# aproposorg/sydr

Measured on AMD Instinct MI355X. Metric: IQ Msamples/s through 32-ch E/P/L correlators @25 MHz fs, higher is better.
Workload: dtype f64

## Files before the change

sydr_amd/csrc/correlator_chip.h:

```cpp
#pragma once

#include "correlator.h"

#pragma clang fp contract(off)

namespace sdr {

constexpr int kChipMax = 26;
constexpr double kChipMinCodeStep = 1.0 / 25.9;
constexpr double kChipMaxCodeStep = 1.0 / 15.5;
constexpr int kChipRawDwords = 13;
constexpr int kChipRotSlots = 2 * kChipMax + 2;
template <int NT>
constexpr int chip_strip_slots() { return 2 * NT + 1; }

__host__ __device__ __forceinline__ int chip_first_above(double thr, double shift, double inv_step, bool& near) {
    const double u = (thr - shift) * inv_step;
    const double fl = floor(u);
    const double fr = u - fl;
    near = near || fr < kNearInteger || fr > 1.0 - kNearInteger;
    return (int)fl + 1;
}
__host__ __device__ __forceinline__ int chip_first_above_exact(int c, double thr, double step, double shift) {
    auto above = [&](int i) {
        double y = (double)i * step;
        y = y + shift;
        return y > thr;
    };
    if (c >= 1 && above(c - 1)) return (c >= 2 && above(c - 2)) ? c - 2 : c - 1;
    if (c < 0) c = 0;
    if (above(c)) return c;
    return above(c + 1) ? c + 1 : c + 2;
}

template <int B, int E, class F>
__device__ __forceinline__ void static_for(F&& f) {
    if constexpr (B < E) {
        f(std::integral_constant<int, B>{});
        static_for<B + 1, E>(f);
    }
}

__device__ __forceinline__ int wave_min_i32(int x) {
#pragma unroll
    for (int off = 1; off < 64; off <<= 1) {
        const int o = __shfl_xor(x, off, 64);
        x = o < x ? o : x;
    }
    return __builtin_amdgcn_readfirstlane(x);
}

#ifndef SDR_BIASED_CVT
#define SDR_BIASED_CVT 1
#endif
constexpr double kCvtBias = 4224.0;
#ifndef SDR_ALT_PAIRS
#define SDR_ALT_PAIRS 1
#endif
typedef uint32_t sdr_u32x2 __attribute__((ext_vector_type(2)));
__device__ __forceinline__ double biased_sample(sdr_u32x2& pair, uint32_t w_flipped, uint32_t selector, uint32_t hi_const) {
    pair.y = __builtin_amdgcn_perm(w_flipped, hi_const, selector);
    return __builtin_bit_cast(double, pair);
}
constexpr uint32_t cvt_selector(int byte) { return 0x03020000u | ((uint32_t)(4 + byte) << 8) | 0x0Cu; }

template <int NT>
struct ChipGeom {
    int64_t Tfx, Ufx;
    uint64_t delta[NT];
    int q0, F;
    int head_end, tail_start;
    int m[NT], J[NT];
    int bad;
};

template <int NT, int KM, int KS, int KI>
__host__ __device__ __forceinline__ void chip_geometry(int n, const double* shift, const double* step, const double* inv_step,
                                                       ChipGeom<NT>& g) {
    constexpr int A = NT / 2;
    const double two32 = 4294967296.0;
    g.q0 = (int)ceil(shift[A]);
    double y_last = (double)(n - 1) * step[A];
    y_last = y_last + shift[A];
    const int q_last = (int)ceil(y_last);
    g.F = q_last - g.q0 - 1;
    g.head_end = n, g.tail_start = n;
    if (g.F > 0) {
        bool nr = false;
        g.head_end = chip_first_above_exact(chip_first_above((double)g.q0, shift[A], inv_step[A], nr), (double)g.q0, step[A], shift[A]);
        g.tail_start = chip_first_above_exact(chip_first_above((double)(q_last - 1), shift[A], inv_step[A], nr),
                                              (double)(q_last - 1), step[A], shift[A]);
    }
    g.Tfx = (int64_t)rint(inv_step[A] * two32);
    g.Ufx = (int64_t)floor(-shift[A] * inv_step[A] * two32);
    const int M = (int)(g.Tfx >> 32);
    bool bad = M < 1 || M + 1 > kChipMax || g.F > 16384 || (KM != 0 && M != KM);
#pragma unroll
    for (int t = 0; t < NT; ++t) {
        g.m[t] = M, g.J[t] = 0, g.delta[t] = 0;
        if (t == A) continue;
        const int64_t Ut = (int64_t)floor(-shift[t] * inv_step[t] * two32);
        int j = (int)ceil(shift[t] - shift[A]) - 1;
        int64_t d = (Ut - g.Ufx) + (int64_t)(1 + j) * g.Tfx;
        if (d < 0) {
            d += g.Tfx;
            ++j;
        } else if (d >= g.Tfx) {
            d -= g.Tfx;
            --j;
        }
        bad = bad || d < 0 || d >= g.Tfx;
        g.J[t] = j;
        g.delta[t] = (uint64_t)d;
        g.m[t] = (int)(d >> 32);
        bad = bad || (KS != 0 && (g.m[t] != KS || j != (t < A ? -1 : 0)));
        bad = bad || (KI != 0 && !((j == (t - A) * KI - 1 && g.m[t] == 0) || (j == (t - A) * KI && g.m[t] >= M)));
    }
    g.bad = bad ? 1 : 0;
}

constexpr int kStaticHalf = 13;
constexpr int chip_half(int KM, int KS, int KI) { return KI != 0 ? (KM + 2) / 2 : KS + 1; }
struct ChipRot {
    double urc[kStaticHalf + 1], urs[kStaticHalf + 1];
    double rd0c, rd0s, rd1c, rd1s;
    double biasc[3], biass[3];
};
__host__ __device__ inline void chip_rotations(double dphi, int Dmin, ChipRot& r, int half = kStaticHalf, int cmin = kStaticHalf - 2) {
    double cs[16], sn[16];
    for (int k = 0; k < 16; ++k) sincos_reduced(-(double)k * dphi, &sn[k], &cs[k]);
    for (int k = 1; k <= half; ++k) r.urc[k] = cs[k], r.urs[k] = sn[k];
    r.urc[0] = 1.0, r.urs[0] = 0.0;
    sincos_reduced(-(double)Dmin * dphi, &r.rd0s, &r.rd0c);
    sincos_reduced(-(double)(Dmin + 1) * dphi, &r.rd1s, &r.rd1c);
    for (int st = 1; st < 16; st <<= 1)
        for (int l = 15; l >= st; --l) cs[l] += cs[l - st], sn[l] += sn[l - st];
    for (int i = 0; i < 3; ++i) {
        const int l = cmin + i - 1;
        const double re = cs[l] - sn[l], im = cs[l] + sn[l];
        r.biasc[i] = re * 4224.0, r.biass[i] = im * 4224.0;
    }
}

template <int NT>
struct ChipSetup {
    double dphi;
    double shift[NT], step[NT], inv_step[NT];
    int64_t base;
    ChipGeom<NT> g;
    ChipRot r;
};

template <int NT, int KM, int KS, int KI>
__host__ __device__ inline void chip_setup(int n, int64_t start_sample, int64_t capacity, double carrier_hz, double rem_code,
                                           double code_step, const double* spacing, double fs, int stride, ChipSetup<NT>& S) {
    S = ChipSetup<NT>{};
    S.dphi = carrier_step(carrier_hz, fs);
    const double nd = (double)n;
    for (int t = 0; t < NT; ++t) {
        const double shift = rem_code + spacing[t];
        double stop = code_step * nd;
        stop = stop + shift;
        const double delta = stop - shift;
        S.shift[t] = shift;
        S.step[t] = delta / nd;
        S.inv_step[t] = 1.0 / S.step[t];
    }
    const int64_t base = start_sample % capacity;
    const bool applies = code_step >= kChipMinCodeStep && code_step <= kChipMaxCodeStep && base + n + 32 <= capacity;
    S.base = applies ? base : -1;
    if (applies) {
        chip_geometry<NT, KM, KS, KI>(n, S.shift, S.step, S.inv_step, S.g);
        chip_rotations(S.dphi, (int)(((int64_t)stride * S.g.Tfx) >> 32), S.r, chip_half(KM, KS, KI), KM - chip_half(KM, KS, KI));
    }
}

struct ChipWalk {
    int S;
    uint32_t f;
};
__host__ __device__ __forceinline__ ChipWalk chip_walk_at(uint64_t u) { return ChipWalk{(int)(u >> 32), (uint32_t)u}; }
__host__ __device__ __forceinline__ bool chip_carry(uint32_t a, uint32_t b, uint32_t& sum) { return __builtin_add_overflow(a, b, &sum); }
__host__ __device__ __forceinline__ bool chip_near_sample(uint32_t fr) { return fr + 0x10000u < 0x20000u; }
__host__ __device__ __forceinline__ bool chip_walk_step(ChipWalk& w, uint32_t stride_lo, int Dmin) {
    const bool dd = chip_carry(w.f, stride_lo, w.f);
    w.S = w.S + Dmin + (dd ? 1 : 0);
    return dd;
}
__host__ __device__ __forceinline__ ChipWalk chip_walk_clamp(const ChipWalk& w, bool inside, const ChipWalk& w_last) {
    return ChipWalk{inside ? w.S : w_last.S, inside ? w.f : w_last.f};
}
template <int NT, int KI>
__host__ __device__ __forceinline__ void chip_walk_flags(uint32_t f, uint32_t T_lo, const uint32_t* delta_lo, bool& dn, bool* ds, bool& near) {
    uint32_t fE;
    dn = chip_carry(f, T_lo, fE);
    near = chip_near_sample(f) || chip_near_sample(fE);
#pragma unroll
    for (int t = 0; t < NT; ++t) {
        ds[t] = false;
        if (t == NT / 2 || KI != 0) continue;
        uint32_t fT;
        ds[t] = chip_carry(f, delta_lo[t], fT);
        near = near || chip_near_sample(fT);
    }
}

template <int NT>
struct ChipBlock {
    uint32_t raw[kChipRawDwords];
    int S;
    int dn;
    int ds[NT];
    uint32_t f;
    int slow;
    int adj;
};

template <int NT, bool SINGLE_WAVE, int KM = 0, int KS = 0, int KI = 0>
__device__ __forceinline__ bool correlate_epoch_chip(const void* __restrict__ ring, const void* __restrict__ ring_flipped, int64_t capacity,
                                                     const EpochParams& ep, double dphi, const EpochConsts<NT>& K,
                                                     const ChipGeom<NT>& G, int64_t base, const ChipRot* R,
                                                     const uint32_t* lut, double2* strip_lds, double2* rot, int tid,
                                                     int lane, int stride, int edge_lane, double* accr, double* acci) {
    constexpr int A = NT / 2;
    constexpr int kSlots = chip_strip_slots<NT>();
    const int n = ep.n;
    const double* shift = K.shift;
    const double* step = K.step;
    double2* strip = strip_lds + tid * kSlots;
    const int wlane = threadIdx.x & 63;
#pragma unroll
    for (int t = 0; t < NT; ++t) accr[t] = acci[t] = 0.0;

    const double dphi_u = uniform(dphi), rem_carrier_u = uniform(ep.rem_carrier);
    const int q0 = __builtin_amdgcn_readfirstlane(G.q0);
    const int F = __builtin_amdgcn_readfirstlane(G.F);
    const int head_end = __builtin_amdgcn_readfirstlane(G.head_end);
    const int tail_start = __builtin_amdgcn_readfirstlane(G.tail_start);
    (void)ring_flipped;
    const char* ring_base = static_cast<const char*>(ring) + base * 2;

    static_assert(!(KS != 0 && KI != 0), "either the taps switch inside the block (KS) or with it (KI)");
    constexpr bool kStatic = KM != 0 && (KS != 0 || KI != 0);
    constexpr bool kWalk = kStatic && (KS != 0 || NT > 3);
    constexpr int kHalf = chip_half(KM, KS, KI);
    double urc[kStatic ? kHalf + 1 : 1], urs[kStatic ? kHalf + 1 : 1];
    double biasc[3] = {0.0, 0.0, 0.0}, biass[3] = {0.0, 0.0, 0.0};
    const double two32 = 4294967296.0;
    int64_t Tfx = G.Tfx;
    int64_t stride_fx = (int64_t)stride * Tfx;
    const int Dmin = (int)(stride_fx >> 32);
    if constexpr (kStatic) asm volatile("" : "+v"(Tfx), "+v"(stride_fx));
    double rd0c = 1.0, rd0s = 0.0, rd1c = 1.0, rd1s = 0.0;
    {
        double sn = 0.0, cs = 0.0;
        if constexpr (kStatic) {
            static_assert(kHalf <= kStaticHalf, "the plan's rotations are laid out for half blocks of up to 13 samples");
#pragma unroll
            for (int k = 1; k <= kHalf; ++k) urc[k] = R->urc[k], urs[k] = R->urs[k];
            rd0c = R->rd0c, rd0s = R->rd0s, rd1c = R->rd1c, rd1s = R->rd1s;
            if constexpr (SDR_BIASED_CVT) {
#pragma unroll
                for (int i = 0; i < 3; ++i) {
                    biasc[i] = R->biasc[i], biass[i] = R->biass[i];
                    if constexpr (kWalk && (kHalf >= 12 || NT > 3)) asm volatile("" : "+v"(biasc[i]), "+v"(biass[i]));
                }
            }
        } else {
            if (wlane < kChipMax) {
                sincos_reduced(-(double)wlane * dphi_u, &sn, &cs);
                rot[wlane] = make_double2(cs, sn);
            }
            if constexpr (SDR_BIASED_CVT) {
                double br = (cs - sn) * kCvtBias, bi = (cs + sn) * kCvtBias;
#pragma unroll
                for (int off = 1; off < 32; off <<= 1) {
                    const double o_r = __shfl_up(br, off, 64), o_i = __shfl_up(bi, off, 64);
                    br = wlane >= off ? br + o_r : br;
                    bi = wlane >= off ? bi + o_i : bi;
                }
                double2* const btab = rot + kChipMax;
                if (wlane < kChipMax) btab[wlane + 1] = make_double2(br, bi);
                if (wlane == 0) btab[0] = make_double2(0.0, 0.0);
            }
        }
    }

    bool bad = false;
    const int rounds = F > 0 ? (F + stride - 1) / stride : 0;
    if (rounds > 0) {
        int64_t Ufx = G.Ufx;
        const int M = (int)(G.Tfx >> 32);
        if constexpr (kStatic) asm volatile("" : "+v"(Ufx));
        bad = bad || G.bad != 0;
        int m[NT], J[NT];
        uint64_t delta[NT];
        unsigned evmask = (1u << M) | (2u << M);
#pragma unroll
        for (int t = 0; t < NT; ++t) {
            m[t] = G.m[t], J[t] = G.J[t], delta[t] = G.delta[t];
            if constexpr (kStatic) asm volatile("" : "+v"(m[t]), "+v"(J[t]), "+v"(delta[t]));
            if (t != A) evmask |= (1u << m[t]) | (2u << m[t]);
        }
        const int k_last = M + 1;
        int rank[NT];
#pragma unroll
        for (int t = 0; t < NT; ++t) rank[t] = __builtin_popcount(evmask & ((1u << m[t]) - 1u));
        if constexpr (!kStatic) {
            double sn, cs;
            sincos_reduced(-(double)(Dmin + (wlane & 1)) * dphi_u, &sn, &cs);
            rd0c = lane_value(cs, 0), rd0s = lane_value(sn, 0);
            rd1c = lane_value(cs, 1), rd1s = lane_value(sn, 1);
        }
        asm volatile("" : "+v"(rd0c), "+v"(rd0s), "+v"(rd1c), "+v"(rd1s));
        const uint64_t lane_fx = (uint64_t)((int64_t)lane * Tfx);
        uint64_t u_cur = (uint64_t)(Ufx + (int64_t)q0 * Tfx + (int64_t)two32) + lane_fx;
        const int last_idx = F - 1;

        auto prepare = [&](int round, uint64_t u0, ChipBlock<NT>& b) {
            const int idx = round * stride + lane;
            const bool inside = idx <= last_idx;
            const uint64_t uS = inside ? u0 : (uint64_t)(Ufx + (int64_t)(q0 + last_idx) * Tfx + (int64_t)two32);
            const uint64_t uE = uS + (uint64_t)Tfx;
            int S = (int)(uS >> 32);
            int E = (int)(uE >> 32);
            bool near = (uint32_t)uS + 0x10000u < 0x20000u || (uint32_t)uE + 0x10000u < 0x20000u;
            int split[NT];
#pragma unroll
            for (int t = 0; t < NT; ++t) {
                split[t] = 0;
                if (t == A) continue;
                if constexpr (KI != 0) {
                    split[t] = J[t] == (t - A) * KI ? E - S : 0;
                    continue;
                }
                const uint64_t uT = uS + delta[t];
                near = near || (uint32_t)uT + 0x10000u < 0x20000u;
                split[t] = (int)(uT >> 32) - S;
            }
            if (__builtin_expect(__any(near), 0)) {
                const int q = q0 + 1 + (inside ? idx : last_idx);
                S = chip_first_above_exact(S, (double)(q - 1), step[A], shift[A]);
                E = chip_first_above_exact(E, (double)q, step[A], shift[A]);
#pragma unroll
                for (int t = 0; t < NT; ++t) {
                    if (t == A) continue;
                    const int p0 = q + J[t];
                    const int bt = chip_first_above_exact(S + split[t], (double)p0, step[t], shift[t]);
                    double y = (double)S * step[t];
                    y = y + shift[t];
                    const int at_s = (int)ceil(y);
                    bad = bad || (at_s != p0 && at_s != p0 + 1) || (at_s == p0 + 1 && bt > S);
                    split[t] = bt < S ? 0 : bt - S;
                }
            }
            b.S = S;
            const int nn = E - S;
            b.dn = nn - M;
            bad = bad || (unsigned)b.dn > 1u;
#pragma unroll
            for (int t = 0; t < NT; ++t) {
                b.ds[t] = 0;
                if (t == A) continue;
                const int sp = split[t] > nn ? nn : split[t];
                if constexpr (KI != 0) {
                    bad = bad || !(J[t] == (t - A) * KI ? sp == nn : sp == 0);
                    continue;
                }
                b.ds[t] = sp - m[t];
                bad = bad || (unsigned)b.ds[t] > 1u;
            }
            if constexpr (KS != 0 && NT == 3) bad = bad || b.ds[0] != b.ds[2];
            const char* src = ring_base + (int64_t)S * 2;
            const uint4 w0 = *reinterpret_cast<const uint4*>(src);
            const uint4 w1 = *reinterpret_cast<const uint4*>(src + 16);
            const uint4 w2 = *reinterpret_cast<const uint4*>(src + 32);
            const uint32_t w3 = *reinterpret_cast<const uint32_t*>(src + 48);
            b.raw[0] = w0.x, b.raw[1] = w0.y, b.raw[2] = w0.z, b.raw[3] = w0.w;
            b.raw[4] = w1.x, b.raw[5] = w1.y, b.raw[6] = w1.z, b.raw[7] = w1.w;
            b.raw[8] = w2.x, b.raw[9] = w2.y, b.raw[10] = w2.z, b.raw[11] = w2.w;
            b.raw[12] = w3;
        };

        const uint32_t T_lo = (uint32_t)Tfx, stride_lo = (uint32_t)stride_fx;
        uint32_t delta_lo[NT];
#pragma unroll
        for (int t = 0; t < NT; ++t) delta_lo[t] = (uint32_t)delta[t];
        int bad_v = 0;
        int Dmin_v = Dmin;
        if constexpr (kWalk) asm volatile("" : "+v"(bad_v), "+v"(Dmin_v));
        auto prepare_walk = [&](auto clampc, int round, const ChipWalk& w_in, ChipBlock<NT>& b) {
            constexpr bool kClamp = decltype(clampc)::value;
            const int idx = round * stride + lane;
            bool inside = true;
            ChipWalk w = w_in;
            if constexpr (kClamp) {
                inside = idx <= last_idx;
                w = chip_walk_clamp(w_in, inside, chip_walk_at((uint64_t)(Ufx + (int64_t)(q0 + last_idx) * Tfx + (int64_t)two32)));
            }
            bool dn, ds[NT], near;
            chip_walk_flags<NT, KI>(w.f, T_lo, delta_lo, dn, ds, near);
            if constexpr (KS != 0 && NT == 3) near = near || ds[0] != ds[2];
            b.f = w.f;
            b.slow = 0;
            uint32_t off;
            if (__builtin_expect(__any(near), 0)) {
                int S = w.S;
                int E = S + M + (dn ? 1 : 0);
                int split[NT];
#pragma unroll
                for (int t = 0; t < NT; ++t) {
                    split[t] = 0;
                    if (t == A) continue;
                    if constexpr (KI != 0)
                        split[t] = J[t] == (t - A) * KI ? E - S : 0;
                    else
                        split[t] = m[t] + (ds[t] ? 1 : 0);
                }
                bool wrong = false;
                const int q = q0 + 1 + (inside ? idx : last_idx);
                S = chip_first_above_exact(S, (double)(q - 1), step[A], shift[A]);
                E = chip_first_above_exact(E, (double)q, step[A], shift[A]);
#pragma unroll
                for (int t = 0; t < NT; ++t) {
                    if (t == A) continue;
                    const int p0 = q + J[t];
                    const int bt = chip_first_above_exact(S + split[t], (double)p0, step[t], shift[t]);
                    double y = (double)S * step[t];
                    y = y + shift[t];
                    const int at_s = (int)ceil(y);
                    wrong = wrong || (at_s != p0 && at_s != p0 + 1) || (at_s == p0 + 1 && bt > S);
                    split[t] = bt < S ? 0 : bt - S;
                }
                const int nn = E - S;
                b.dn = nn - M;
                wrong = wrong || (unsigned)b.dn > 1u;
#pragma unroll
                for (int t = 0; t < NT; ++t) {
                    b.ds[t] = 0;
                    if (t == A) continue;
                    const int sp = split[t] > nn ? nn : split[t];
                    if constexpr (KI != 0) {
                        wrong = wrong || !(J[t] == (t - A) * KI ? sp == nn : sp == 0);
                        continue;
                    }
                    b.ds[t] = sp - m[t];
                    wrong = wrong || (unsigned)b.ds[t] > 1u;
                }
                if constexpr (KS != 0 && NT == 3) wrong = wrong || b.ds[0] != b.ds[2];
                bad_v |= wrong ? 1 : 0;
                b.adj = S - w.S;
                b.slow = 1;
                off = (uint32_t)S << 1;
            } else {
                off = (uint32_t)w.S << 1;
            }
            asm volatile("" : "+s"(b.slow));
            const char* src = ring_base + off;
            const uint4 w0 = *reinterpret_cast<const uint4*>(src);
            const uint4 w1 = *reinterpret_cast<const uint4*>(src + 16);
            const uint4 w2 = *reinterpret_cast<const uint4*>(src + 32);
            const uint32_t w3 = *reinterpret_cast<const uint32_t*>(src + 48);
            b.raw[0] = w0.x, b.raw[1] = w0.y, b.raw[2] = w0.z, b.raw[3] = w0.w;
            b.raw[4] = w1.x, b.raw[5] = w1.y, b.raw[6] = w1.z, b.raw[7] = w1.w;
            b.raw[8] = w2.x, b.raw[9] = w2.y, b.raw[10] = w2.z, b.raw[11] = w2.w;
            b.raw[12] = w3;
        };

        ChipBlock<NT> blk_a, blk_b;
        ChipWalk walk = chip_walk_at(u_cur);
        if constexpr (kWalk) {
            prepare_walk(std::true_type{}, 0, walk, blk_a);
            const ChipWalk w0 = chip_walk_clamp(walk, lane <= last_idx, chip_walk_at((uint64_t)(Ufx + (int64_t)(q0 + last_idx) * Tfx + (int64_t)two32)));
            blk_a.S = w0.S + (blk_a.slow ? blk_a.adj : 0);
        } else {
            prepare(0, u_cur, blk_a);
        }
        double sb, cb;
        sincos_reduced(__builtin_fma(-(double)blk_a.S, dphi_u, rem_carrier_u), &sb, &cb);
        if constexpr (!kStatic) {
            sb = lane <= last_idx ? sb : 0.0;
            cb = lane <= last_idx ? cb : 0.0;
        }
        const int q_lane = q0 + 1 + lane + SDR_LUT_PAD;
        const uint32_t* zero_lq = reinterpret_cast<const uint32_t*>(strip) + 3;
        if constexpr (kStatic) strip[0] = strip[1] = make_double2(0.0, 0.0);

        sdr_u32x2 zI = {0u, 0u}, zQ = {0u, 0u};
        asm volatile("" : "+v"(zI), "+v"(zQ));
        sdr_u32x2 zI2 = {0u, 0u}, zQ2 = {0u, 0u};
        if constexpr (kWalk) asm volatile("" : "+v"(zI2), "+v"(zQ2));

        uint32_t hi_epoch = 0x40B00000u;
        if constexpr (kWalk && SDR_BIASED_CVT) asm volatile("" : "+v"(hi_epoch));
        auto process = [&](const ChipBlock<NT>& b, int round, double sbk, double cbk, auto clampc) {
            constexpr bool kClamp = decltype(clampc)::value;
            double pr = 0.0, pi = 0.0;
            double2* wp = strip;
            unsigned evm = evmask;
            int klast = k_last;
            if constexpr (!kStatic) asm volatile("" : "+s"(evm), "+s"(klast));
            constexpr int kAhead = 4;
            double2 rr[kChipMax + kAhead];
            if constexpr (!kStatic) {
#pragma unroll
                for (int k = 0; k < kAhead; ++k) rr[k] = rot[k];
            }
            auto park = [&]() {
                *wp = make_double2(pr, pi);
                ++wp;
                asm volatile("" ::: "memory");
            };
            uint32_t hi_rt = 0x40B00000u;
            uint32_t sel_rt[4] = {cvt_selector(0), cvt_selector(1), cvt_selector(2), cvt_selector(3)};
            if constexpr (!kStatic && SDR_BIASED_CVT) {
                asm volatile("" : "+v"(hi_rt));
                asm volatile("" : "+s"(sel_rt[0]), "+s"(sel_rt[1]), "+s"(sel_rt[2]), "+s"(sel_rt[3]));
            }
            auto sample = [&](auto kc) {
                constexpr int k = decltype(kc)::value;
                double ar, ai;
                if constexpr (SDR_BIASED_CVT) {
                    ar = biased_sample(zI, b.raw[k >> 1], sel_rt[(k & 1) ? 2 : 0], hi_rt);
                    ai = biased_sample(zQ, b.raw[k >> 1], sel_rt[(k & 1) ? 3 : 1], hi_rt);
                } else {
                    const int w = ci8_native((int)b.raw[k >> 1]);
                    ar = (k & 1) ? (double)(int)(int8_t)(w >> 16) : (double)(int)(int8_t)w;
                    ai = (k & 1) ? (double)(w >> 24) : (double)(int)(int8_t)(w >> 8);
                }
                if (k + kAhead < kChipMax) rr[k + kAhead] = rot[k + kAhead];
                const double2 r = rr[k];
                pr = __builtin_fma(-ai, r.y, __builtin_fma(ar, r.x, pr));
                pi = __builtin_fma(ai, r.x, __builtin_fma(ar, r.y, pi));
                if constexpr (SDR_BIASED_CVT) asm volatile("" : "+v"(pr), "+v"(pi), "+v"(zI), "+v"(zQ));
            };
            double capr[3] = {0.0, 0.0, 0.0}, capi[3] = {0.0, 0.0, 0.0};
            if constexpr (kStatic) {
                static_assert(2 * kHalf >= KM + 1 && kHalf < KM, "two halves of at most KS + 1 samples cover the block");
                static_assert(!SDR_BIASED_CVT || (2 * kHalf - KM >= 1 && 2 * kHalf - KM <= 2 && (KS == 0 || KS == kHalf - 1)),
                              "the offset's shares are kept for sums of KM - kHalf, + 1 and + 2 samples: kHalf must be one of the last two");
                uint32_t flipped[kChipRawDwords];
                uint32_t hi_const = hi_epoch;
                if constexpr (SDR_BIASED_CVT) {
                    if constexpr (!kWalk) asm volatile("" : "+v"(hi_const));
#pragma unroll
                    for (int i = 0; i < kChipRawDwords; ++i) flipped[i] = b.raw[i];
                }
                static_for<0, KM + 1>([&](auto kc) {
                    constexpr int k = decltype(kc)::value;
                    constexpr int j = k < kHalf ? k : k - kHalf;
                    const int w = ci8_native((int)b.raw[k >> 1]);
                    double ar, ai;
                    if constexpr (SDR_BIASED_CVT) {
                        ar = biased_sample(kWalk && SDR_ALT_PAIRS && (k & 1) ? zI2 : zI, flipped[k >> 1], cvt_selector((k & 1) ? 2 : 0), hi_const);
                        ai = biased_sample(kWalk && SDR_ALT_PAIRS && (k & 1) ? zQ2 : zQ, flipped[k >> 1], cvt_selector((k & 1) ? 3 : 1), hi_const);
                    } else {
                        ar = (k & 1) ? (double)(int)(int8_t)(w >> 16) : (double)(int)(int8_t)w;
                        ai = (k & 1) ? (double)(w >> 24) : (double)(int)(int8_t)(w >> 8);
                    }
                    if constexpr (KS != 0 && k == KS) capr[0] = pr, capi[0] = pi;
                    if constexpr (k == KM) capr[1] = pr, capi[1] = pi;
                    if constexpr (k == kHalf) capr[2] = pr, capi[2] = pi;
                    if constexpr (j == 0) {
                        pr = ar, pi = ai;
                    } else {
                        pr = __builtin_fma(-ai, urs[j], __builtin_fma(ar, urc[j], pr));
                        pi = __builtin_fma(ai, urc[j], __builtin_fma(ar, urs[j], pi));
                    }
                    if constexpr (SDR_BIASED_CVT) {
                        if constexpr (kWalk && SDR_ALT_PAIRS && (k & 1)) asm volatile("" : "+v"(pr), "+v"(pi), "+v"(zI2), "+v"(zQ2));
                        else asm volatile("" : "+v"(pr), "+v"(pi), "+v"(zI), "+v"(zQ));
                    }
                });
            } else if constexpr (KM != 0) {
                static_for<0, KM>([&](auto kc) {
                    constexpr int k = decltype(kc)::value;
                    if (evm & (1u << k)) park();
                    sample(kc);
                });
                park();
                sample(std::integral_constant<int, KM>{});
                park();
            } else {
#pragma unroll
                for (int k = 0; k <= kChipMax; ++k) {
                    if (evm & (1u << k)) {
                        park();
                        if (k == klast) break;
                    }
                    if (k < kChipMax) {
                        double ar, ai;
                        if constexpr (SDR_BIASED_CVT) {
                            ar = biased_sample(zI, b.raw[k >> 1], sel_rt[(k & 1) ? 2 : 0], hi_rt);
                            ai = biased_sample(zQ, b.raw[k >> 1], sel_rt[(k & 1) ? 3 : 1], hi_rt);
                        } else {
                            const int w = ci8_native((int)b.raw[k >> 1]);
                            ar = (k & 1) ? (double)(int)(int8_t)(w >> 16) : (double)(int)(int8_t)w;
                            ai = (k & 1) ? (double)(w >> 24) : (double)(int)(int8_t)(w >> 8);
                        }
                        if (k + kAhead < kChipMax) rr[k + kAhead] = rot[k + kAhead];
                        const double2 r = rr[k];
                        pr = __builtin_fma(-ai, r.y, __builtin_fma(ar, r.x, pr));
                        pi = __builtin_fma(ai, r.x, __builtin_fma(ar, r.y, pi));
                        if constexpr (SDR_BIASED_CVT) asm volatile("" : "+v"(pr), "+v"(pi), "+v"(zI), "+v"(zQ));
                    }
                }
            }
            double2 ptot;
            if constexpr (kStatic && SDR_BIASED_CVT) {
                constexpr int iFirst = 2 * kHalf - KM;
                pr -= biasc[1], pi -= biass[1];
                capr[1] -= biasc[0], capi[1] -= biass[0];
                capr[2] -= biasc[iFirst], capi[2] -= biass[iFirst];
                if constexpr (KS != 0) capr[0] -= biasc[iFirst - 1], capi[0] -= biass[iFirst - 1];
            }
            bool dnf = false, dsf[NT];
#pragma unroll
            for (int t = 0; t < NT; ++t) dsf[t] = false;
            if constexpr (kWalk) {
                if (__builtin_expect(b.slow != 0, 0)) {
                    dnf = b.dn != 0;
#pragma unroll
                    for (int t = 0; t < NT; ++t) dsf[t] = b.ds[t] != 0;
                    asm volatile("" : "+v"(pr), "+v"(pi));
                } else {
                    uint32_t f = b.f;
                    asm volatile("" : "+v"(f), "+v"(pr), "+v"(pi));
                    bool nr;
                    chip_walk_flags<NT, KI>(f, T_lo, delta_lo, dnf, dsf, nr);
                }
            }
            if constexpr (kStatic) {
                if constexpr (!kWalk) dnf = b.dn != 0;
                const double qr = dnf ? pr : capr[1], qi = dnf ? pi : capi[1];
                ptot.x = __builtin_fma(-qi, urs[kHalf], __builtin_fma(qr, urc[kHalf], capr[2]));
                ptot.y = __builtin_fma(qi, urc[kHalf], __builtin_fma(qr, urs[kHalf], capi[2]));
            } else {
                ptot = strip[rank[A] + b.dn];
                if constexpr (SDR_BIASED_CVT) {
                    const double2 bb = (rot + kChipMax)[M + b.dn];
                    ptot.x -= bb.x, ptot.y -= bb.y;
                }
            }
            const int first = round * stride;
            const uint32_t* lq;
            if constexpr (kStatic)
                lq = !kClamp || first + lane <= last_idx ? lut + q_lane + first : zero_lq;
            else
                lq = lut + q_lane + (first + lane <= last_idx ? first : last_idx - lane);
            if constexpr (KI != 0) {
                const double xr = __builtin_fma(-sbk, ptot.y, cbk * ptot.x);
                const double xi = __builtin_fma(sbk, ptot.x, cbk * ptot.y);
#pragma unroll
                for (int t = 0; t < NT; ++t) {
                    const double c = __hiloint2double((int)lq[(t - A) * KI], 0);
                    accr[t] = __builtin_fma(c, xr, accr[t]);
                    acci[t] = __builtin_fma(c, xi, acci[t]);
                }
                return;
            }
#pragma unroll
            for (int t = 0; t < NT; ++t) {
                double gr, gi;
                if (t == A) {
                    const double c = __hiloint2double((int)lq[0], 0);
                    gr = c * ptot.x;
                    gi = c * ptot.y;
                } else {
                    double2 ps;
                    if constexpr (kStatic)
                        ps = (kWalk ? dsf[NT == 3 ? 0 : t] : b.ds[NT == 3 ? 0 : t] != 0) ? make_double2(capr[2], capi[2]) : make_double2(capr[0], capi[0]);
                    else {
                        ps = strip[rank[t] + b.ds[t]];
                        if constexpr (SDR_BIASED_CVT) {
                            const double2 bb = (rot + kChipMax)[m[t] + b.ds[t]];
                            ps.x -= bb.x, ps.y -= bb.y;
                        }
                    }
                    const int jt = kStatic ? (t < A ? -1 : 0) : J[t];
                    const double ca = __hiloint2double((int)lq[jt], 0);
                    const double cbn = __hiloint2double((int)lq[jt + 1], 0);
                    const double diff = ca - cbn;
                    gr = __builtin_fma(diff, ps.x, cbn * ptot.x);
                    gi = __builtin_fma(diff, ps.y, cbn * ptot.y);
                }
                accr[t] = __builtin_fma(-sbk, gi, __builtin_fma(cbk, gr, accr[t]));
                acci[t] = __builtin_fma(sbk, gr, __builtin_fma(cbk, gi, acci[t]));
            }
        };

        auto wave_has_work = [&](int round) { return SINGLE_WAVE || round * stride + (lane - wlane) <= last_idx; };
        auto advance = [&](const ChipBlock<NT>& from, const ChipBlock<NT>& to, int to_round) {
            const unsigned dd = (unsigned)(to.S - from.S - Dmin);
            const bool alive = to_round * stride + lane <= last_idx;
            bad = bad || (alive && dd > 1u);
            const double rc_ = dd ? rd1c : rd0c, rs_ = dd ? rd1s : rd0s;
            const double cbn = __builtin_fma(cb, rc_, -sb * rs_);
            const double sbn = __builtin_fma(sb, rc_, cb * rs_);
            if constexpr (kStatic) {
                cb = cbn, sb = sbn;
            } else {
                cb = alive ? cbn : 0.0;
                sb = alive ? sbn : 0.0;
            }
        };

        static_assert(SINGLE_WAVE || !kWalk, "the straight-line forms give a wave an epoch of its own");
        if constexpr (kWalk) {
            auto next_block = [&](auto clampc, const ChipBlock<NT>& from, ChipBlock<NT>& to, int to_round) {
                constexpr bool kClamp = decltype(clampc)::value;
                bool dd = chip_walk_step(walk, stride_lo, Dmin_v);
                prepare_walk(clampc, to_round, walk, to);
                if (__builtin_expect((from.slow | to.slow) != 0, 0)) {
                    bool alive = true;
                    int d = dd ? 1 : 0;
                    if constexpr (kClamp) {
                        alive = to_round * stride + lane <= last_idx;
                        const int S_last = (int)((uint64_t)(Ufx + (int64_t)(q0 + last_idx) * Tfx + (int64_t)two32) >> 32);
                        d = alive ? d : S_last - (walk.S - d - Dmin_v) - Dmin_v;
                    }
                    if (to.slow) d += to.adj;
                    if (from.slow) d -= from.adj;
                    bad_v |= alive && (unsigned)d > 1u ? 1 : 0;
                    dd = d != 0;
                    asm volatile("");
                }
                const double rc_ = dd ? rd1c : rd0c, rs_ = dd ? rd1s : rd0s;
                const double cbn = __builtin_fma(cb, rc_, -sb * rs_);
                const double sbn = __builtin_fma(sb, rc_, cb * rs_);
                cb = cbn, sb = sbn;
                asm volatile("" : "+v"(cb), "+v"(sb));
            };
            auto settle = [&]() {
#pragma unroll
                for (int t = 0; t < NT; ++t) asm volatile("" : "+v"(accr[t]), "+v"(acci[t]));
            };
            auto round_pair = [&](auto clampc, int it) {
                const double sb0 = sb, cb0 = cb;
                next_block(clampc, blk_a, blk_b, 2 * it + 1);
                process(blk_a, 2 * it, sb0, cb0, clampc);
                settle();
                const double sb1 = sb, cb1 = cb;
                if (!decltype(clampc)::value || 2 * it + 2 < rounds) next_block(clampc, blk_b, blk_a, 2 * it + 2);
                process(blk_b, 2 * it + 1, sb1, cb1, clampc);
                settle();
            };
            const int plain = rounds >= 2 ? (rounds - 2) / 2 : 0;
            for (int it = 0; it < plain; ++it) round_pair(std::false_type{}, it);
            for (int it = plain; it < rounds / 2; ++it) round_pair(std::true_type{}, it);
            if (rounds & 1) process(blk_a, rounds - 1, sb, cb, std::true_type{});
        } else {
            for (int it = 0; it < rounds / 2; ++it) {
                const double sb0 = sb, cb0 = cb;
                u_cur += (uint64_t)stride_fx;
                prepare(2 * it + 1, u_cur, blk_b);
                advance(blk_a, blk_b, 2 * it + 1);
                if (wave_has_work(2 * it)) process(blk_a, 2 * it, sb0, cb0, std::true_type{});
                const double sb1 = sb, cb1 = cb;
                if (2 * it + 2 < rounds) {
                    u_cur += (uint64_t)stride_fx;
                    prepare(2 * it + 2, u_cur, blk_a);
                    advance(blk_b, blk_a, 2 * it + 2);
                }
                if (wave_has_work(2 * it + 1)) process(blk_b, 2 * it + 1, sb1, cb1, std::true_type{});
            }
            if ((rounds & 1) && wave_has_work(rounds - 1)) process(blk_a, rounds - 1, sb, cb, std::true_type{});
        }
        bad = bad || bad_v != 0;
    }

    if (__any(bad)) return false;
    if (edge_lane >= 0) {
        if (head_end + (n - tail_start) > 64) {
            for (int off = 0; off < head_end + (n - tail_start); off += 64)
                edge_samples<SDR_FMT_CI8, NT>(ring, capacity, ep, dphi, shift, step, lut, edge_lane + off, head_end, tail_start, accr, acci, base);
        } else {
            edge_samples<SDR_FMT_CI8, NT>(ring, capacity, ep, dphi, shift, step, lut, edge_lane, head_end, tail_start, accr, acci, base);
        }
    }
    return true;
}

__device__ __forceinline__ bool chip_variant_applies(const EpochParams& ep, int64_t capacity) {
    return ep.code_step >= kChipMinCodeStep && ep.code_step <= kChipMaxCodeStep &&
           ep.start_sample % capacity + ep.n + 32 <= capacity;
}

}
```

sydr_amd/csrc/epl_kernel.h:

```cpp
#pragma once
#include "correlator.h"
#include "correlator_chip.h"

namespace {

using namespace sdr;

constexpr int kWaveThreads = 64;
constexpr int kVariantKS12 = 256 * 12;
constexpr int kVariantKSMask = 256 * 15;
constexpr int kVariantKS9 = 256 * 9;
constexpr int kVariantKM1516 = 16;
constexpr int kVariantKI = 4096;
constexpr int kVariantC2 = 8192;
constexpr int kLongLutWords = 4096;

#ifndef SDR_EPL_WAVES
#define SDR_EPL_WAVES 1
#endif
template <int FMT, int NT, int W, int KM = 0, int WPW = 1, int KS = 0, int KI = 0, int KM2 = 0>
#ifndef SDR_EPL_KS_WAVES
#define SDR_EPL_KS_WAVES 3
#endif
#ifndef SDR_EPL_KI_WAVES
#define SDR_EPL_KI_WAVES 1
#endif
#ifndef SDR_EPL_KM2_WAVES
#define SDR_EPL_KM2_WAVES 1
#endif
__global__ __launch_bounds__(kWaveThreads * WPW, (KS != 0 ? SDR_EPL_KS_WAVES : (KI != 0 ? SDR_EPL_KI_WAVES : (KM2 != 0 ? SDR_EPL_KM2_WAVES : SDR_EPL_WAVES)))) void epl_kernel(const void* __restrict__ ring, const void* __restrict__ ring_flipped, int64_t capacity,
                                                       const sdr_epl_item* __restrict__ items, int n_items, int group_stride,
                                                       const uint32_t* __restrict__ luts,
                                                       int lut_words, int lut_stride,
                                                       const double* __restrict__ spacing, double fs,
                                                       int tap0, int n_taps_total,
                                                       double* __restrict__ out, const void* __restrict__ setups) {
    constexpr int kThreads = kWaveThreads * WPW;
    constexpr bool kPre = W == kChipMax && FMT == SDR_FMT_CI8 && KM != 0 && (KS != 0 || KI != 0);
    extern __shared__ double smem[];
    double* red = smem;
    double2* prefix = reinterpret_cast<double2*>(red + WPW * 2 * NT);
    constexpr int kScratchSlots = W == kChipMax ? kThreads * chip_strip_slots<NT>() + WPW * kChipRotSlots : (W ? kThreads * kPrefixSlots : 0);
    uint32_t* lut = reinterpret_cast<uint32_t*>(prefix + kScratchSlots);

    const int tid = threadIdx.x;
    const int wave = __builtin_amdgcn_readfirstlane(tid >> 6), lane = tid & 63;
#ifdef SDR_TRACE_WG
    const unsigned long long t_start = wall_clock64();
#endif
    int item = blockIdx.x;
    if (WPW > 1) {
        const int g = blockIdx.x / group_stride, c = blockIdx.x - g * group_stride;
        item = (g * WPW + wave) * group_stride + c;
    }
    const bool have = item < n_items;
    const int column = (int)(blockIdx.x % group_stride);
    const sdr_epl_item it = items[have ? item : (column < n_items ? column : n_items - 1)];
    stage_lut<kThreads>(lut, luts + (size_t)it.code_slot * lut_stride, lut_words, tid);
    double dphi;
    if constexpr (!kPre) dphi = carrier_step(it.carrier_hz, fs);
    EpochParams ep;
    ep.start_sample = it.start_sample;
    ep.n = it.n_samples;
    ep.carrier_hz = it.carrier_hz;
    ep.rem_carrier = it.rem_carrier;
    ep.rem_code = it.rem_code;
    ep.code_step = it.code_step;
    EpochConsts<NT> K;
    ChipGeom<NT> G;
    const ChipRot* rot_plan = nullptr;
    int64_t base = -1;
    if constexpr (kPre) {
        const ChipSetup<NT>& S = static_cast<const ChipSetup<NT>*>(setups)[have ? item : 0];
        dphi = S.dphi;
#pragma unroll
        for (int q = 0; q < NT; ++q) {
            K.shift[q] = S.shift[q], K.step[q] = S.step[q], K.inv_step[q] = S.inv_step[q];
            asm volatile("" : "+v"(K.shift[q]), "+v"(K.step[q]), "+v"(K.inv_step[q]));
        }
        G = S.g;
        rot_plan = &S.r;
        base = S.base;
    } else if constexpr (W == kChipMax && FMT == SDR_FMT_CI8) {
        compute_tap_constants<NT>(K, ep, spacing + tap0);
        if (chip_variant_applies(ep, capacity)) {
            base = ep.start_sample % capacity;
            chip_geometry<NT, (KM2 != 0 ? 0 : KM), KS, KI>(ep.n, K.shift, K.step, K.inv_step, G);
        }
    } else {
        compute_constants<NT>(K, ep, spacing + tap0, dphi, kWaveThreads);
    }
    __syncthreads();
    if (WPW > 1 && !have) return;

    double accr[NT], acci[NT];
    if constexpr (W == kChipMax && FMT == SDR_FMT_CI8) {
        bool done = false;
        if constexpr (KM2 != 0) {
            static_assert(KS == 0 && KI == 0 && !kPre, "two block lengths: tap positions at run time, no plan setups");
            const int M = __builtin_amdgcn_readfirstlane((int)(G.Tfx >> 32));
            double2* const rot = prefix + kThreads * chip_strip_slots<NT>() + wave * kChipRotSlots;
            if (base >= 0 && M == KM)
                done = correlate_epoch_chip<NT, true, KM, 0, 0>(ring, ring_flipped, capacity, ep, dphi, K, G, base, rot_plan, lut, prefix, rot,
                                                                 tid, lane, kWaveThreads, lane, accr, acci);
            else if (base >= 0 && M == KM2)
                done = correlate_epoch_chip<NT, true, KM2, 0, 0>(ring, ring_flipped, capacity, ep, dphi, K, G, base, rot_plan, lut, prefix, rot,
                                                                  tid, lane, kWaveThreads, lane, accr, acci);
        } else {
            done = base >= 0 &&
                   correlate_epoch_chip<NT, true, KM, KS, KI>(ring, ring_flipped, capacity, ep, dphi, K, G, base, rot_plan, lut, prefix,
                                                              prefix + kThreads * chip_strip_slots<NT>() + wave * kChipRotSlots,
                                                              tid, lane, kWaveThreads, lane, accr, acci);
        }
        if (!done) {
            EpochConsts<NT> K2;
            compute_constants<NT>(K2, ep, spacing + tap0, dphi, kWaveThreads);
            correlate_epoch<FMT, NT>(ring, capacity, ep, dphi, K2, lut, lane, kWaveThreads, lane, accr, acci);
        }
    } else if (W != 0 && !epoch_wraps(ep, capacity))
        correlate_epoch_wide<FMT, NT, true, (W ? W : kWide)>(ring, capacity, ep, dphi, K, lut, prefix, tid, lane, kWaveThreads, lane, accr, acci);
    else
        correlate_epoch<FMT, NT>(ring, capacity, ep, dphi, K, lut, lane, kWaveThreads, lane, accr, acci);
    if constexpr (NT == 3 || NT == 5) {
        int slot;
        const double total = reduce_taps_scatter<NT>(accr, acci, lane, slot);
        if (lane < (NT == 3 ? 8 : 16)) out[(size_t)item * 2 * n_taps_total + 2 * tap0 + slot] = total;
    } else {
        const double total = reduce_taps<NT, kWaveThreads>(accr, acci, red, lane);
        if (lane < 2 * NT) out[(size_t)item * 2 * n_taps_total + 2 * tap0 + lane] = total;
    }
#ifdef SDR_TRACE_WG
    if (tid == 0 && blockIdx.x < 65536) {
        unsigned hw;
        asm volatile("s_getreg_b32 %0, hwreg(HW_REG_HW_ID)" : "=s"(hw));
        unsigned xcc;
        asm volatile("s_getreg_b32 %0, hwreg(HW_REG_XCC_ID)" : "=s"(xcc));
        g_wg_trace[3 * blockIdx.x] = t_start;
        g_wg_trace[3 * blockIdx.x + 1] = wall_clock64();
        g_wg_trace[3 * blockIdx.x + 2] = ((unsigned long long)xcc << 32) | hw;
    }
#endif
}

}
```

Before: 97790.

## Fold symmetric sample pairs around block centre to halve carrier rotation multiplies

Within each static chip block, samples are paired symmetrically about the run centre. Their sum and difference are formed with packed udot4 byte conversions, so one cosine/sine pair rotates two samples at once. The carrier reference moves to the run centre, and new per-plan constants (pair rotations, tail rotations, bias corrections) are precomputed in the setup struct. The aim is fewer FMAs and conversions per sample, at the cost of more setup state, more registers and new bias-correction bookkeeping.

```diff
diff --git a/sydr_amd/csrc/correlator_chip.h b/sydr_amd/csrc/correlator_chip.h
--- a/sydr_amd/csrc/correlator_chip.h
+++ b/sydr_amd/csrc/correlator_chip.h
@@ -142,6 +142,43 @@
     }
 }
 
+#ifndef SDR_FOLD_PAIRS
+#define SDR_FOLD_PAIRS 1
+#endif
+constexpr int kFoldPairsMax = kStaticHalf / 2;
+constexpr double kFoldSumBias = 8192.0 + 256.0, kFoldDiffBias = 8192.0 + 255.0;
+constexpr int chip_fold_first(int half, int h) { return h == 0 ? 0 : half; }
+constexpr int chip_fold_count(int KM, int half, bool ks, int h) { return h == 0 ? (ks ? half - 1 : half) : KM - half; }
+struct ChipFold {
+    double pc[2][kFoldPairsMax], ps[2][kFoldPairsMax];
+    double sc[2], ss[2];
+    double tc, ts;
+    double shc[4], shs[4];
+};
+__host__ __device__ inline void chip_fold_constants(double dphi, int KM, int half, bool ks, ChipFold& f) {
+    f = ChipFold{};
+    for (int h = 0; h < 2; ++h) {
+        const int count = chip_fold_count(KM, half, ks, h);
+        double re = (count & 1) ? kCvtBias : 0.0, im = re;
+        for (int i = 0; i < count / 2; ++i) {
+            const double d = 0.5 * (double)(count - 1 - 2 * i);
+            sincos_reduced(d * dphi, &f.ps[h][i], &f.pc[h][i]);
+            re += f.pc[h][i] * kFoldSumBias - f.ps[h][i] * kFoldDiffBias;
+            im += f.pc[h][i] * kFoldSumBias + f.ps[h][i] * kFoldDiffBias;
+        }
+        sincos_reduced(-0.5 * (double)(count + 1) * dphi, &f.ss[h], &f.sc[h]);
+        f.shc[2 * h] = re, f.shs[2 * h] = im;
+        f.shc[2 * h + 1] = re + (f.sc[h] - f.ss[h]) * kCvtBias, f.shs[2 * h + 1] = im + (f.sc[h] + f.ss[h]) * kCvtBias;
+    }
+    const double turn = (double)chip_fold_first(half, 1) + 0.5 * (double)(chip_fold_count(KM, half, ks, 1) - 1) -
+                        0.5 * (double)(chip_fold_count(KM, half, ks, 0) - 1);
+    sincos_reduced(-turn * dphi, &f.ts, &f.tc);
+}
+constexpr bool chip_folds(int NT, int KM, int KS, int KI) {
+    return SDR_FOLD_PAIRS != 0 && SDR_BIASED_CVT != 0 && KM != 0 && (KS != 0 || KI != 0) &&
+           (NT > 3 || (KS != 0 ? KM >= 20 : KM <= 17));
+}
+
 template <int NT>
 struct ChipSetup {
     double dphi;
@@ -149,6 +186,9 @@
     int64_t base;
     ChipGeom<NT> g;
     ChipRot r;
+#if SDR_FOLD_PAIRS
+    ChipFold f;
+#endif
 };
 
 template <int NT, int KM, int KS, int KI>
@@ -172,6 +212,9 @@
     if (applies) {
         chip_geometry<NT, KM, KS, KI>(n, S.shift, S.step, S.inv_step, S.g);
         chip_rotations(S.dphi, (int)(((int64_t)stride * S.g.Tfx) >> 32), S.r, chip_half(KM, KS, KI), KM - chip_half(KM, KS, KI));
+#if SDR_FOLD_PAIRS
+        if constexpr (chip_folds(NT, KM, KS, KI)) chip_fold_constants(S.dphi, KM, chip_half(KM, KS, KI), KS != 0, S.f);
+#endif
     }
 }
 
@@ -221,7 +264,8 @@
                                                      const EpochParams& ep, double dphi, const EpochConsts<NT>& K,
                                                      const ChipGeom<NT>& G, int64_t base, const ChipRot* R,
                                                      const uint32_t* lut, double2* strip_lds, double2* rot, int tid,
-                                                     int lane, int stride, int edge_lane, double* accr, double* acci) {
+                                                     int lane, int stride, int edge_lane, double* accr, double* acci,
+                                                     const ChipFold* RF = nullptr) {
     constexpr int A = NT / 2;
     constexpr int kSlots = chip_strip_slots<NT>();
     const int n = ep.n;
@@ -244,6 +288,10 @@
     constexpr bool kStatic = KM != 0 && (KS != 0 || KI != 0);
     constexpr bool kWalk = kStatic && (KS != 0 || NT > 3);
     constexpr int kHalf = chip_half(KM, KS, KI);
+    constexpr bool kFold = kStatic && chip_folds(NT, KM, KS, KI);
+    constexpr int kFoldN0 = chip_fold_count(KM, kHalf, KS != 0, 0), kFoldN1 = chip_fold_count(KM, kHalf, KS != 0, 1);
+    double fpc[2][kFoldPairsMax], fps[2][kFoldPairsMax], fsc[2] = {1.0, 1.0}, fss[2] = {0.0, 0.0};
+    double fshc[4] = {0.0, 0.0, 0.0, 0.0}, fshs[4] = {0.0, 0.0, 0.0, 0.0};
     double urc[kStatic ? kHalf + 1 : 1], urs[kStatic ? kHalf + 1 : 1];
     double biasc[3] = {0.0, 0.0, 0.0}, biass[3] = {0.0, 0.0, 0.0};
     const double two32 = 4294967296.0;
@@ -256,10 +304,27 @@
         double sn = 0.0, cs = 0.0;
         if constexpr (kStatic) {
             static_assert(kHalf <= kStaticHalf, "the plan's rotations are laid out for half blocks of up to 13 samples");
-#pragma unroll
-            for (int k = 1; k <= kHalf; ++k) urc[k] = R->urc[k], urs[k] = R->urs[k];
+            if constexpr (kFold) {
+                static_assert(kFoldN0 / 2 <= kFoldPairsMax && kFoldN1 / 2 <= kFoldPairsMax, "the plan's pair rotations are laid out for runs of up to 13 samples");
+#pragma unroll
+                for (int h = 0; h < 2; ++h) {
+#pragma unroll
+                    for (int i = 0; i < (h == 0 ? kFoldN0 : kFoldN1) / 2; ++i) fpc[h][i] = RF->pc[h][i], fps[h][i] = RF->ps[h][i];
+                    if (h == 1 || KS != 0) fsc[h] = RF->sc[h], fss[h] = RF->ss[h];
+                }
+                urc[kHalf] = RF->tc, urs[kHalf] = RF->ts;
+#pragma unroll
+                for (int i = 0; i < 4; ++i) {
+                    if (i == 1 && KS == 0) continue;
+                    fshc[i] = RF->shc[i], fshs[i] = RF->shs[i];
+                    if constexpr (kWalk && (kHalf >= 12 || NT > 3)) asm volatile("" : "+v"(fshc[i]), "+v"(fshs[i]));
+                }
+            } else {
+#pragma unroll
+                for (int k = 1; k <= kHalf; ++k) urc[k] = R->urc[k], urs[k] = R->urs[k];
+            }
             rd0c = R->rd0c, rd0s = R->rd0s, rd1c = R->rd1c, rd1s = R->rd1s;
-            if constexpr (SDR_BIASED_CVT) {
+            if constexpr (SDR_BIASED_CVT && !kFold) {
 #pragma unroll
                 for (int i = 0; i < 3; ++i) {
                     biasc[i] = R->biasc[i], biass[i] = R->biass[i];
@@ -477,7 +542,11 @@
             prepare(0, u_cur, blk_a);
         }
         double sb, cb;
-        sincos_reduced(__builtin_fma(-(double)blk_a.S, dphi_u, rem_carrier_u), &sb, &cb);
+        constexpr double kRefSample = kFold ? 0.5 * (double)(kFoldN0 - 1) : 0.0;
+        if constexpr (kFold)
+            sincos_reduced(__builtin_fma(-((double)blk_a.S + kRefSample), dphi_u, rem_carrier_u), &sb, &cb);
+        else
+            sincos_reduced(__builtin_fma(-(double)blk_a.S, dphi_u, rem_carrier_u), &sb, &cb);
         if constexpr (!kStatic) {
             sb = lane <= last_idx ? sb : 0.0;
             cb = lane <= last_idx ? cb : 0.0;
@@ -489,10 +558,13 @@
         sdr_u32x2 zI = {0u, 0u}, zQ = {0u, 0u};
         asm volatile("" : "+v"(zI), "+v"(zQ));
         sdr_u32x2 zI2 = {0u, 0u}, zQ2 = {0u, 0u};
-        if constexpr (kWalk) asm volatile("" : "+v"(zI2), "+v"(zQ2));
+        if constexpr (kWalk || kFold) asm volatile("" : "+v"(zI2), "+v"(zQ2));
+        sdr_u32x2 zDI = {0u, 0u}, zDQ = {0u, 0u}, zDI2 = {0u, 0u}, zDQ2 = {0u, 0u};
+        uint32_t hi_fold = 0x40C00000u;
+        if constexpr (kFold) asm volatile("" : "+v"(zDI), "+v"(zDQ), "+v"(zDI2), "+v"(zDQ2), "+v"(hi_fold));
 
         uint32_t hi_epoch = 0x40B00000u;
-        if constexpr (kWalk && SDR_BIASED_CVT) asm volatile("" : "+v"(hi_epoch));
+        if constexpr ((kWalk || kFold) && SDR_BIASED_CVT) asm volatile("" : "+v"(hi_epoch));
         auto process = [&](const ChipBlock<NT>& b, int round, double sbk, double cbk, auto clampc) {
             constexpr bool kClamp = decltype(clampc)::value;
             double pr = 0.0, pi = 0.0;
@@ -542,10 +614,73 @@
                 uint32_t flipped[kChipRawDwords];
                 uint32_t hi_const = hi_epoch;
                 if constexpr (SDR_BIASED_CVT) {
-                    if constexpr (!kWalk) asm volatile("" : "+v"(hi_const));
+                    if constexpr (!kWalk && !kFold) asm volatile("" : "+v"(hi_const));
 #pragma unroll
                     for (int i = 0; i < kChipRawDwords; ++i) flipped[i] = b.raw[i];
                 }
+                if constexpr (kFold) {
+                    auto single = [&](auto kc, auto seqc, bool start, double rc, double rs) {
+                        constexpr int k = decltype(kc)::value;
+                        constexpr bool alt = SDR_ALT_PAIRS && (decltype(seqc)::value & 1);
+                        const double ar = biased_sample(alt ? zI2 : zI, flipped[k >> 1], cvt_selector((k & 1) ? 2 : 0), hi_const);
+                        const double ai = biased_sample(alt ? zQ2 : zQ, flipped[k >> 1], cvt_selector((k & 1) ? 3 : 1), hi_const);
+                        if (start) {
+                            pr = ar, pi = ai;
+                        } else {
+                            pr = __builtin_fma(-ai, rs, __builtin_fma(ar, rc, pr));
+                            pi = __builtin_fma(ai, rc, __builtin_fma(ar, rs, pi));
+                        }
+                        if constexpr (alt) asm volatile("" : "+v"(pr), "+v"(pi), "+v"(zI2), "+v"(zQ2));
+                        else asm volatile("" : "+v"(pr), "+v"(pi), "+v"(zI), "+v"(zQ));
+                    };
+                    auto pair = [&](auto kac, auto kbc, auto seqc, bool start, double c, double sn) {
+                        constexpr int ka = decltype(kac)::value, kb = decltype(kbc)::value;
+                        constexpr bool alt = SDR_ALT_PAIRS && (decltype(seqc)::value & 1);
+                        constexpr uint32_t ia = 4u + 2u * (ka & 1), ib = 2u * (kb & 1);
+                        const uint32_t g = __builtin_amdgcn_perm(flipped[ka >> 1], flipped[kb >> 1], ((ib + 1u) << 24) | (ib << 16) | ((ia + 1u) << 8) | ia);
+                        const uint32_t g2 = g ^ 0xFFFF0000u;
+                        sdr_u32x2& SI = alt ? zI2 : zI;
+                        sdr_u32x2& SQ = alt ? zQ2 : zQ;
+                        sdr_u32x2& DI = alt ? zDI2 : zDI;
+                        sdr_u32x2& DQ = alt ? zDQ2 : zDQ;
+                        SI.y = __builtin_amdgcn_udot4(g, 0x00800080u, hi_fold, false);
+                        SQ.y = __builtin_amdgcn_udot4(g, 0x80008000u, hi_fold, false);
+                        DI.y = __builtin_amdgcn_udot4(g2, 0x00800080u, hi_fold, false);
+                        DQ.y = __builtin_amdgcn_udot4(g2, 0x80008000u, hi_fold, false);
+                        const double si = __builtin_bit_cast(double, SI), sq = __builtin_bit_cast(double, SQ);
+                        const double di = __builtin_bit_cast(double, DI), dq = __builtin_bit_cast(double, DQ);
+                        if (start) {
+                            pr = __builtin_fma(-sn, dq, c * si);
+                            pi = __builtin_fma(sn, di, c * sq);
+                        } else {
+                            pr = __builtin_fma(-sn, dq, __builtin_fma(c, si, pr));
+                            pi = __builtin_fma(sn, di, __builtin_fma(c, sq, pi));
+                        }
+                        if constexpr (alt) asm volatile("" : "+v"(pr), "+v"(pi), "+v"(zI2), "+v"(zQ2), "+v"(zDI2), "+v"(zDQ2));
+                        else asm volatile("" : "+v"(pr), "+v"(pi), "+v"(zI), "+v"(zQ), "+v"(zDI), "+v"(zDQ));
+                    };
+                    static_for<0, 2>([&](auto hc) {
+                        constexpr int h = decltype(hc)::value;
+                        constexpr int first = chip_fold_first(kHalf, h), count = h == 0 ? kFoldN0 : kFoldN1;
+                        constexpr int odd = count & 1;
+                        constexpr int seq0 = h == 0 ? 0 : (kFoldN0 & 1) + kFoldN0 / 2 + (KS != 0 ? 1 : 0);
+                        if constexpr (odd) single(std::integral_constant<int, first + count / 2>{}, std::integral_constant<int, seq0>{}, true, 1.0, 0.0);
+                        static_for<0, count / 2>([&](auto ic) {
+                            constexpr int i = decltype(ic)::value;
+                            pair(std::integral_constant<int, first + i>{}, std::integral_constant<int, first + count - 1 - i>{},
+                                 std::integral_constant<int, seq0 + odd + i>{}, !odd && i == 0, fpc[h][i], fps[h][i]);
+                        });
+                        if constexpr (h == 0) {
+                            capr[0] = pr, capi[0] = pi;
+                            if constexpr (KS != 0)
+                                single(std::integral_constant<int, first + count>{}, std::integral_constant<int, seq0 + odd + count / 2>{}, false, fsc[0], fss[0]);
+                            capr[2] = pr, capi[2] = pi;
+                        } else {
+                            capr[1] = pr, capi[1] = pi;
+                            single(std::integral_constant<int, first + count>{}, std::integral_constant<int, seq0 + odd + count / 2>{}, false, fsc[1], fss[1]);
+                        }
+                    });
+                } else
                 static_for<0, KM + 1>([&](auto kc) {
                     constexpr int k = decltype(kc)::value;
                     constexpr int j = k < kHalf ? k : k - kHalf;
@@ -607,7 +742,12 @@
                 }
             }
             double2 ptot;
-            if constexpr (kStatic && SDR_BIASED_CVT) {
+            if constexpr (kFold) {
+                pr -= fshc[3], pi -= fshs[3];
+                capr[1] -= fshc[2], capi[1] -= fshs[2];
+                capr[2] -= fshc[KS != 0 ? 1 : 0], capi[2] -= fshs[KS != 0 ? 1 : 0];
+                if constexpr (KS != 0) capr[0] -= fshc[0], capi[0] -= fshs[0];
+            } else if constexpr (kStatic && SDR_BIASED_CVT) {
                 constexpr int iFirst = 2 * kHalf - KM;
                 pr -= biasc[1], pi -= biass[1];
                 capr[1] -= biasc[0], capi[1] -= biass[0];
diff --git a/sydr_amd/csrc/epl_kernel.h b/sydr_amd/csrc/epl_kernel.h
--- a/sydr_amd/csrc/epl_kernel.h
+++ b/sydr_amd/csrc/epl_kernel.h
@@ -69,6 +69,7 @@
     EpochConsts<NT> K;
     ChipGeom<NT> G;
     const ChipRot* rot_plan = nullptr;
+    const ChipFold* fold_plan = nullptr;
     int64_t base = -1;
     if constexpr (kPre) {
         const ChipSetup<NT>& S = static_cast<const ChipSetup<NT>*>(setups)[have ? item : 0];
@@ -80,6 +81,9 @@
         }
         G = S.g;
         rot_plan = &S.r;
+#if SDR_FOLD_PAIRS
+        fold_plan = &S.f;
+#endif
         base = S.base;
     } else if constexpr (W == kChipMax && FMT == SDR_FMT_CI8) {
         compute_tap_constants<NT>(K, ep, spacing + tap0);
@@ -105,12 +109,12 @@
                                                                  tid, lane, kWaveThreads, lane, accr, acci);
             else if (base >= 0 && M == KM2)
                 done = correlate_epoch_chip<NT, true, KM2, 0, 0>(ring, ring_flipped, capacity, ep, dphi, K, G, base, rot_plan, lut, prefix, rot,
-                                                                  tid, lane, kWaveThreads, lane, accr, acci);
+                                                                  tid, lane, kWaveThreads, lane, accr, acci, fold_plan);
         } else {
             done = base >= 0 &&
                    correlate_epoch_chip<NT, true, KM, KS, KI>(ring, ring_flipped, capacity, ep, dphi, K, G, base, rot_plan, lut, prefix,
                                                               prefix + kThreads * chip_strip_slots<NT>() + wave * kChipRotSlots,
-                                                              tid, lane, kWaveThreads, lane, accr, acci);
+                                                              tid, lane, kWaveThreads, lane, accr, acci, fold_plan);
         }
         if (!done) {
             EpochConsts<NT> K2;
```

Result: faster. 101,800 (median of 6 runs) (+4.1%).
